# jonasrothfuss/ProMP

Measured on AMD Instinct MI355X. Metric: env-steps/sec through GAE+inner+outer update, higher is better.
Workload: dtype f32

## Files before the change

include/promp_hip.h:

```cpp
#ifndef PROMP_HIP_H
#define PROMP_HIP_H

#include <stddef.h>
#include <stdint.h>

#ifdef __cplusplus
extern "C" {
#endif

typedef struct promp_ctx promp_ctx;

typedef struct promp_dims {
    int32_t n_tasks;
    int32_t n_tasks_global;
    int32_t obs_dim;
    int32_t act_dim;
    int32_t hidden1, hidden2;
    int32_t num_inner_steps;
    int32_t max_rows;
    int32_t max_paths;
    int32_t n_hidden;
    int32_t hidden3, hidden4;
    int32_t hidden_act;
} promp_dims;
// ... 57 lines not shown
int promp_set_theta(promp_ctx* ctx, const float* theta);
int promp_get_theta(promp_ctx* ctx, float* theta);
int promp_set_step_sizes(promp_ctx* ctx, const float* step_sizes);
int promp_get_step_sizes(promp_ctx* ctx, float* step_sizes);
int promp_set_train_step_sizes(promp_ctx* ctx, int on);
int promp_get_step_size_grad(promp_ctx* ctx, float* grad);
int promp_set_step_size_adam_state(promp_ctx* ctx, const float* m, const float* v);
int promp_get_step_size_adam_state(promp_ctx* ctx, float* m, float* v);
int promp_set_learn_std(promp_ctx* ctx, int learn_std);
int promp_set_min_std(promp_ctx* ctx, float min_std);
int promp_set_schedule(promp_ctx* ctx, int stage_overlap, int fuse_min_tasks);
int promp_set_primal_cache(promp_ctx* ctx, int on);
int promp_set_reuse_adapt(promp_ctx* ctx, int on);
long long promp_adapt_passes_skipped(promp_ctx* ctx);
long long promp_constraint_hvp_cached_passes(promp_ctx* ctx);
long long promp_state_version(promp_ctx* ctx);
int promp_set_adam_state(promp_ctx* ctx, const float* m, const float* v, int64_t t);
int promp_get_adam_state(promp_ctx* ctx, float* m, float* v, int64_t* t);
int promp_switch_to_pre_update(promp_ctx* ctx);
int promp_set_task_thetas(promp_ctx* ctx, const float* theta_tasks);
int promp_get_task_thetas(promp_ctx* ctx, float* theta_tasks);

int promp_inner_adapt(promp_ctx* ctx, int step, int inner_kind);

int promp_policy_forward(promp_ctx* ctx, const float* obs, int batch, float* mean_out);

int promp_begin_rollout(promp_ctx* ctx, int step, int envs_per_task, int path_length);
int promp_begin_collection(promp_ctx* ctx, int step, int envs_per_task, int max_steps);
int promp_end_collection(promp_ctx* ctx, int step, int n_paths, const int32_t* task_path_offsets, const int32_t* path_env,
                         const int32_t* path_start, const int32_t* path_len, const float* rewards);
// ... 59 lines not shown
```

promp_amd/_lib.py:

```python
import ctypes as C
import os

import weakref

import numpy as np

_HERE = os.path.dirname(os.path.abspath(__file__))
DEFAULT_LIBRARY = os.path.join(_HERE, 'libpromp_hip.so')

BASELINE_ZERO, BASELINE_LINEAR_FEATURE, BASELINE_LINEAR_TIME = 0, 1, 2
INNER_RATIO, INNER_LOGLIK, INNER_DICE = 0, 1, 2
OUTER_CLIP, OUTER_RATIO, OUTER_KL, OUTER_LOGLIK = 0, 1, 2, 3
LOSS_RATIO, LOSS_CLIP, LOSS_LOGLIK, LOSS_KL = 0, 1, 2, 3
KERNEL_FWD_BWD, KERNEL_HVP, KERNEL_GRAM, KERNEL_FWD, KERNEL_EXCHANGE = 0, 1, 2, 3, 4


class PrompError(RuntimeError):
    pass


class Dims(C.Structure):
    _fields_ = [('n_tasks', C.c_int32), ('n_tasks_global', C.c_int32), ('obs_dim', C.c_int32), ('act_dim', C.c_int32),
                ('hidden1', C.c_int32), ('hidden2', C.c_int32), ('num_inner_steps', C.c_int32),
                ('max_rows', C.c_int32), ('max_paths', C.c_int32),
# ... 34 lines not shown
    'promp_predict_baseline': (C.c_int, [_P, C.c_int, C.c_int, _D]),
    'promp_set_advantages': (C.c_int, [_P, C.c_int, _F]),
    'promp_set_theta': (C.c_int, [_P, _F]),
    'promp_get_theta': (C.c_int, [_P, _F]),
    'promp_set_step_sizes': (C.c_int, [_P, _F]),
    'promp_get_step_sizes': (C.c_int, [_P, _F]),
    'promp_set_train_step_sizes': (C.c_int, [_P, C.c_int]),
    'promp_get_step_size_grad': (C.c_int, [_P, _F]),
    'promp_set_step_size_adam_state': (C.c_int, [_P, _F, _F]),
    'promp_get_step_size_adam_state': (C.c_int, [_P, _F, _F]),
    'promp_set_learn_std': (C.c_int, [_P, C.c_int]),
    'promp_set_primal_cache': (C.c_int, [_P, C.c_int]),
    'promp_set_reuse_adapt': (C.c_int, [_P, C.c_int]),
    'promp_adapt_passes_skipped': (C.c_longlong, [_P]),
    'promp_constraint_hvp_cached_passes': (C.c_longlong, [_P]),
    'promp_state_version': (C.c_longlong, [_P]),
    'promp_set_min_std': (C.c_int, [_P, C.c_float]),
    'promp_set_schedule': (C.c_int, [_P, C.c_int, C.c_int]),
    'promp_set_rewards_f64': (C.c_int, [_P, C.c_int, _D]),
    'promp_stage_step': (C.c_int, [_P, C.c_int, C.c_int, _I, _I, _F, _F, _F, _F, _F, C.c_int]),
    'promp_commit_step': (C.c_int, [_P, C.c_int]),
    'promp_stage_wait': (C.c_int, [_P]),
    'promp_host_alloc': (C.c_void_p, [C.c_size_t]),
    'promp_host_free': (None, [C.c_void_p]),
    'promp_constraint_hvp': (C.c_int, [_P, C.c_int, _F, C.c_int, _F]),
    'promp_cg_solve': (C.c_int, [_P, C.c_int, _F, C.c_int, C.c_float, C.c_float, C.c_int, C.c_float, _F, C.POINTER(C.c_double)]),
    'promp_set_step_selection': (C.c_int, [_P, C.c_int, C.c_int, _I]),
    'promp_step_selection': (C.c_int, [_P, C.c_int]),
    'promp_use_selection': (C.c_int, [_P, C.c_int]),
    'promp_set_adam_state': (C.c_int, [_P, _F, _F, C.c_int64]),
# ... 657 lines not shown
    def set_primal_cache(self, on=True):
        self._call('promp_set_primal_cache', -1 if on is None else int(bool(on)))

    def set_reuse_adapt(self, on=True):
        self._call('promp_set_reuse_adapt', int(bool(on)))

    def adapt_passes_skipped(self):
        return int(self.lib.cdll.promp_adapt_passes_skipped(self._h))

    def state_version(self):
        return int(self.lib.cdll.promp_state_version(self._h))

    def constraint_hvp_cached_passes(self):
        return int(self.lib.cdll.promp_constraint_hvp_cached_passes(self._h))

    def set_min_std(self, min_std):
        self._call('promp_set_min_std', float(min_std))

    def set_learn_std(self, on=True):
        self._call('promp_set_learn_std', int(bool(on)))

    def adam_step(self, lr):
        self._call('promp_adam_step', float(lr))

    def optimize(self, num_epochs, lr, clip_eps, inner_kl_coeff, inner_kind=INNER_RATIO, outer_kind=OUTER_CLIP):
        eta = _f32(inner_kl_coeff)
        assert eta.shape == (self.K,)
        lb, stats = C.c_float(0), np.empty(self.K + 2, np.float32)
        self._call('promp_optimize', int(num_epochs), float(lr), float(clip_eps), _ptr(eta, C.c_float), int(inner_kind),
                   int(outer_kind), C.byref(lb), _ptr(stats, C.c_float))
# ... 166 lines not shown
```

promp_amd/csrc/promp_hip.hip:

```cpp
#include "promp_plan.h"
#include "promp_kernels_chain.h"
#include "promp_kernels_pass.h"
#include "promp_kernels_policy.h"
#include "promp_kernels_policy_wide.h"
#include "promp_kernels_wide_bf16.h"
#include "promp_kernels_sample.h"
#include "promp_kernels_rollout.h"
#include "promp_kernels_generic.h"
#include "promp_kernels_generic_bf16.h"
#include "../../include/promp_hip.h"

#include <algorithm>
#include <cmath>
#include <cstdarg>
#include <cstdio>
#include <cstdlib>
#include <cstring>
#include <memory>
#include <string>
#include <vector>

#define PROMP_ARCH_NAME(prop) (prop).gcnArchName

namespace {
// ... 195 lines not shown
    float eta_last[PROMP_ETA_MAX] = {};
    DevBuf<double> gram_partials, red64;
    DevBuf<char> rollout_buf;
    DevBuf<float> stage_rows;
    DevBuf<double> fit_scratch;
    size_t smem_fwd = 0, smem_hvp = 0;
    PlanSwitches sw;
    PassFamily family = PassFamily::Chain;
    int wb_cls = 0;
    size_t smem_wb_fwd = 0, smem_wb_bwd = 0, smem_wb_hvp = 0;
    DevBuf<unsigned> wb_planes, wb_vplanes;
    DevBuf<unsigned> wb_planes_meta;
    DevBuf<float> cg_buf;
    DevBuf<double> cg_scal;
    struct { bool valid = false; unsigned long long theta_version = 0, data_version = 0, sizes_version = 0; const void* step = nullptr; } wbp;
    DevBuf<unsigned> vdir_absmax;
    int gramt_map_nblk = -1;
    GramtMap gramt_map;
    bool gen_bf16 = true;
    DevBuf<unsigned short> gb_wplanes, gb_vplanes;
    long long gb_plane_stride = 0;
    int gb_pf_off[GEN_MAX_LIN] = {}, gb_pb_off[GEN_MAX_LIN] = {};
    int n_lin = 0, g_maxw = 0;
    GenLin lin[GEN_MAX_LIN];
    DevBuf<float> g_act[GEN_MAX_LIN], g_ract[GEN_MAX_LIN], g_mu, g_rmu, g_dz[2], g_qz[2];
    DevBuf<unsigned long long> dbg;
    bool dbg_enabled = false;
    DevBuf<int> task_counters;
    DevBuf<int> split_events;
    ncclComm_t comm = nullptr;
// ... 228 lines not shown
    const int slices = (c->n_cus * 2 + c->d.n_tasks - 1) / c->d.n_tasks;
    PROMP_LAUNCH(k_obs_range, dim3(slices < 1 ? 1 : slices > 32 ? 32 : slices, c->d.n_tasks), 256, 16, st, r);
    HIPCHECK(hipGetLastError());
    S.obs_range_valid = true;
    c->wbp.valid = false;
    return 0;
}

static bool primal_cache_on(const promp_ctx* c) { return c->family == PassFamily::Chain && c->primal_cache != 0; }
static int ensure_primal_cache(promp_ctx* c, StepData& S) {
    if (S.hcache) return 0;
    const size_t rows = S.cap_rows ? S.cap_rows : c->d.max_rows;
    return S.hcache.alloc((rows + 16 * (size_t)c->d.n_tasks) * chain_cache_row(c->d.hidden1, c->d.hidden2));
}

static void launch_chain(promp_ctx* c, StepData& S, const PassArgs& a, const PassReq& q, int cache) {
    const int n1 = c->d.hidden1 / 16, n2 = c->d.hidden2 / 16, ks = chain_ksteps(c->d.obs_dim);
    const dim3 grid(S.n_chain_wg);
    if (q.hvp) {
#define PROMP_CHAIN_CASE(N1, N2, KS)                                                                                             \
    if (n1 == N1 && n2 == N2 && ks == KS) {                                                                                      \
        if (cache == 2) { auto k = k_chain_hvp<N1, N2, KS, CHAIN_NW_HVP, true>; PROMP_LAUNCH(k, grid, 64 * CHAIN_NW_HVP, c->smem_hvp, c->stream, a); } \
        else { auto k = k_chain_hvp<N1, N2, KS, CHAIN_NW_HVP, false>; PROMP_LAUNCH(k, grid, 64 * CHAIN_NW_HVP, c->smem_hvp, c->stream, a); }           \
    }
        PROMP_CHAIN_ALL(PROMP_CHAIN_CASE)
#undef PROMP_CHAIN_CASE
        return;
    }
#define PROMP_PASS_CASE(N1, N2)                                                                                                          \
    if (n1 == N1 && n2 == N2) {                                                                                                          \
        if (q.fwd_only) { auto k = k_pass<N1, N2, CHAIN_NW_HVP, false, false>; PROMP_LAUNCH(k, grid, 64 * CHAIN_NW_HVP, c->smem_fwd, c->stream, a); }   \
        else if (cache == 1) { auto k = k_pass<N1, N2, CHAIN_NW_HVP, true, true>; PROMP_LAUNCH(k, grid, 64 * CHAIN_NW_HVP, c->smem_fwd, c->stream, a); } \
        else { auto k = k_pass<N1, N2, CHAIN_NW_HVP, true, false>; PROMP_LAUNCH(k, grid, 64 * CHAIN_NW_HVP, c->smem_fwd, c->stream, a); }            \
    }
    PROMP_PASS_ALL(PROMP_PASS_CASE)
#undef PROMP_PASS_CASE
}

static void launch_coop_fp32(promp_ctx* c, StepData& S, const PassArgs& a, const PassReq& q) {
    const int nob = wide_nob(c->d.obs_dim);
    const size_t sm = q.hvp ? c->smem_hvp : c->smem_fwd;
#define PROMP_WIDE_CASE(HH, NOB)                                                                                                \
    if (c->d.hidden1 == HH && nob == NOB) {                                                                                      \
        if (q.hvp) { auto k = k_wide_hvp<HH, NOB>; PROMP_LAUNCH(k, dim3(S.n_work[0]), 4 * HH, sm, c->stream, a); }               \
        else if (q.fwd_only) { auto k = k_wide_fwd_bwd<HH, NOB, false>; PROMP_LAUNCH(k, dim3(S.n_work[0]), 4 * HH, sm, c->stream, a); } \
        else { auto k = k_wide_fwd_bwd<HH, NOB, true>; PROMP_LAUNCH(k, dim3(S.n_work[0]), 4 * HH, sm, c->stream, a); }            \
    }
    PROMP_WIDE_ALL(PROMP_WIDE_CASE)
#undef PROMP_WIDE_CASE
}
// ... 53 lines not shown
    a.segs = S.chain_segs; a.wg_seg_offsets = S.chain_wg_offsets;
    a.theta = q.theta; a.theta_task_stride = q.theta_stride;
    a.vdir = c->vbuf;
    a.partials = c->partials; a.partial_stride = c->partial_stride;
    a.O = c->d.obs_dim; a.A = c->d.act_dim;
    a.loss_kind = q.loss_kind; a.clip_eps = q.clip_eps; a.clip_log_std = q.clip_ls;
    a.min_log_std = c->min_log_std;
    a.kl_weight = q.klw;
    a.task_counters = c->task_counters; a.task_slot_offsets = S.chain_slot_offsets;
    a.fuse_reduce = (q.hvp && chain && c->d.n_tasks >= c->fuse_min_tasks) ? 1 : 0;
    float* scal = q.scal ? q.scal : c->scal_tmp;
    a.red_mode = q.red_mode; a.step_sizes = c->step_sizes; a.cur = q.cur; a.cur_task_stride = q.cur_stride; a.next = q.next;
    a.lam = c->lam; a.v = c->vbuf; a.scal = scal;
    a.dbg = c->dbg_enabled ? c->dbg.p : nullptr;
    a.split_events = c->split_events;
    const int id = q.hvp ? PROMP_KERNEL_HVP : q.fwd_only ? PROMP_KERNEL_FWD : PROMP_KERNEL_FWD_BWD;
    if (prof_begin(c, id, S.n_rows)) return -2;
    switch (c->family) {
    case PassFamily::Chain: launch_chain(c, S, a, q, cache); break;
    case PassFamily::CoopFp32: launch_coop_fp32(c, S, a, q); break;
    case PassFamily::CoopSplit: launch_coop_split(c, S, a, q); break;
    case PassFamily::Layered: if (launch_pass_generic(c, S, a, q.hvp, q.fwd_only)) return -2; break;
    }
    HIPCHECK(hipGetLastError());
    if (prof_end(c, id)) return -2;
    if (a.fuse_reduce) return 0;
    ReduceArgs r;
    r.partials = c->partials; r.partial_stride = c->partial_stride;
    r.task_wg_offsets = chain ? S.chain_slot_offsets : S.task_wg_offsets[0];
    r.NP = c->NP;
// ... 139 lines not shown
    ad.stats = c->stats + (size_t)c->stats_slot * (K + 2); ad.NP = NP; ad.K = K; ad.A = c->d.act_dim;
    for (int k = 0; k < PROMP_ETA_MAX; ++k) ad.eta[k] = k < K ? eta_host[k] : 0.f;
    ad.host_stats = c->publish_next ? c->stats_host.p : nullptr; ad.host_seq = c->stats_seq_host; ad.seq = c->stats_seq;
    ad.inv_tasks = 1.0f / (float)c->d.n_tasks_global;
    ad.do_update = do_adam ? 1 : 0;
    ad.n_trainable = c->learn_std ? NP : NP - c->d.act_dim;
    ad.lr_t = 0.f;
    if (do_adam) {
        c->theta_version = ++c->version_counter;
        if (ag) c->sizes_version = ++c->version_counter;
        c->ls_known = false;
        c->adam_t += 1;
        const double t = (double)c->adam_t;
        ad.lr_t = (float)((double)lr * std::sqrt(1.0 - std::pow(0.999, t)) / (1.0 - std::pow(0.9, t)));
    }
    if (ag) {
        const StepSizeArgs ss = step_size_args(c);
        if (split) PROMP_LAUNCH(k_mean_adam_ss, dim3((2 * NP + 1 + 255) / 256), 256, 0, c->stream, ad, ss);
        else PROMP_LAUNCH(k_final_adam_ss, dim3(final_blocks + 1), 256, 0, c->stream, f, ad, ss);
    } else if (split) PROMP_LAUNCH(k_mean_adam, dim3((NP + 1 + 255) / 256), 256, 0, c->stream, ad);
    else PROMP_LAUNCH(k_final_adam, dim3(final_blocks + 1), 256, 0, c->stream, f, ad);
    HIPCHECK(hipGetLastError());
    for (int k = 0; k <= K; ++k) W[k].dirty = true;
    return 0;
}
int enqueue_meta(promp_ctx* c, float clip_eps, const float* eta_host, int inner_kind, int outer_kind, bool want_grad,
                 bool do_adam, float lr, bool sizes_grad = true) {
    return enqueue_meta_on(c, full_set(c), clip_eps, eta_host, inner_kind, outer_kind, want_grad, do_adam, lr, sizes_grad);
}

// ... 197 lines not shown
        c->smem_fwd = sizeof(float) * (size_t)pass_layout(dims->hidden1 / 16, dims->hidden2 / 16, CHAIN_NW_HVP, c->NP).total;
        c->smem_hvp = sizeof(float) * (size_t)std::max(chain_layout(dims->hidden1 / 16, dims->hidden2 / 16, CHAIN_NW_HVP, true, c->NP).total,
                                                       chain_layout(dims->hidden1 / 16, dims->hidden2 / 16, CHAIN_NW_HVP, true, c->NP, true).total);
        break;
    }
    if (c->smem_hvp > 160 * 1024 || c->smem_fwd > 160 * 1024) {
        const size_t need = c->smem_hvp > c->smem_fwd ? c->smem_hvp : c->smem_fwd;
        return fail(-1, "LDS budget exceeded (%zu bytes)", need);
    }
    {
        const int lds = 160 * 1024;
#define PROMP_CHAIN_LDS(N1, N2, KS) if (allow_lds(lds, k_chain_hvp<N1, N2, KS, CHAIN_NW_HVP, false>, k_chain_hvp<N1, N2, KS, CHAIN_NW_HVP, true>)) return -2;
        PROMP_CHAIN_ALL(PROMP_CHAIN_LDS)
#undef PROMP_CHAIN_LDS
#define PROMP_PASS_LDS(N1, N2) \
    if (allow_lds(lds, k_pass<N1, N2, CHAIN_NW_HVP, true, true>, k_pass<N1, N2, CHAIN_NW_HVP, true, false>, k_pass<N1, N2, CHAIN_NW_HVP, false, false>)) return -2;
        PROMP_PASS_ALL(PROMP_PASS_LDS)
#undef PROMP_PASS_LDS
#define PROMP_WB_LDS(CLS, NKO, NXB) if (allow_lds(lds, k_wb_hvp<NKO, NXB>, k_wb_fwd_bwd<NKO, NXB, true>, k_wb_fwd_bwd<NKO, NXB, false>)) return -2;
        PROMP_WB_ALL(PROMP_WB_LDS)
#undef PROMP_WB_LDS
#define PROMP_WIDE_LDS(HH, NOB) if (allow_lds(lds, k_wide_fwd_bwd<HH, NOB, true>, k_wide_fwd_bwd<HH, NOB, false>, k_wide_hvp<HH, NOB>)) return -2;
        PROMP_WIDE_ALL(PROMP_WIDE_LDS)
#undef PROMP_WIDE_LDS
#define PROMP_GEN_LDS(NBW)                                                                                                   \
    if (allow_lds(lds, k_gen_linear<GEN_FWD, NBW>, k_gen_linear<GEN_FWD_T, NBW>, k_gen_linear<GEN_BWD, NBW>, k_gen_linear<GEN_BWD_T, NBW>, \
                  k_gen_wgrad<1, NBW>, k_gen_wgrad<2, NBW>, k_gb_linear<GEN_FWD, NBW>, k_gb_linear<GEN_FWD_T, NBW>,            \
                  k_gb_linear<GEN_BWD, NBW>, k_gb_linear<GEN_BWD_T, NBW>, k_gb_wgrad<1, NBW>, k_gb_wgrad<2, NBW>)) return -2;
        PROMP_GEN_LDS(1) PROMP_GEN_LDS(2) PROMP_GEN_LDS(3) PROMP_GEN_LDS(4)
#undef PROMP_GEN_LDS
        if (allow_lds((int)gen_loss_smem(GEN_MAX_A), k_gen_loss<true, true>, k_gen_loss<false, true>, k_gen_loss<false, false>)) return -2;
#define PROMP_GRAM_INST(NBLK) k_gram<NBLK>,
#define PROMP_FITWV_INST(DT) k_fit_wave<DT>,
        if (allow_lds(lds, PROMP_GRAM_ALL(PROMP_GRAM_INST) PROMP_FITWV_ALL(PROMP_FITWV_INST) k_fit, k_gram_wide, k_gram_tiled<GRAMT_TB, GRAMT_NWV, GRAMT_NLD>, k_fitw_panel<32>, k_fitw_panel<16>,
                      k_fitw_update<32>, k_fitw_update<16>, k_fitw_back<32>, k_fitw_back<16>, k_fit_wide<32>, k_fit_wide<16>)) return -2;
#undef PROMP_GRAM_INST
#undef PROMP_FITWV_INST
    }
    const size_t NP = c->NP, MNP = (size_t)M * NP;
    if (c->theta.alloc(NP) || c->step_sizes.alloc(NP)) return -2;
    if (c->adam_m.alloc(NP) || c->adam_v.alloc(NP)) return -2;
    if (c->theta_tasks.alloc(MNP) || c->chain.alloc((size_t)(K + 1) * MNP)) return -2;
    if (c->lam.alloc(MNP) || c->vbuf.alloc(MNP)) return -2;
    if (c->family == PassFamily::CoopSplit) {
        const size_t pw = (size_t)M * wb_planes_words(wb_nko(c->wb_cls));
        if (c->wb_planes.alloc(pw) || c->wb_vplanes.alloc(pw) || c->wb_planes_meta.alloc(pw)) return -2;
        if (c->vdir_absmax.alloc((size_t)M)) return -2;
    }
    if (c->partials.alloc((size_t)c->max_work * c->partial_stride)) return -2;
    if (c->scal_inner.alloc((size_t)K * M * 2) || c->scal_outer.alloc((size_t)M * 2)) return -2;
    if (c->scal_tmp.alloc((size_t)M * 2)) return -2;
    if (c->red.alloc(NP + K + 2) || c->grad_mean.alloc(NP)) return -2;
    if (c->stats.alloc((size_t)2 * (K + 2))) return -2;
    if (c->red64.alloc(64)) return -2;
    if (c->family == PassFamily::Layered) {
        const size_t R = (size_t)dims->max_rows;
        for (int l = 1; l < c->n_lin; ++l)
            if (c->g_act[l].alloc(R * c->lin[l].K) || c->g_ract[l].alloc(R * c->lin[l].K)) return -2;
// ... 540 lines not shown
    if (stage_overlap >= 0) {
        HIPCHECK(hipStreamSynchronize(c->side));
        c->overlap = stage_overlap != 0;
    }
    if (fuse_min_tasks >= 0) c->fuse_min_tasks = fuse_min_tasks;
    return 0;
}
int promp_set_reuse_adapt(promp_ctx* c, int on) {
    NEED_CTX(c);
    c->reuse_adapt = on != 0;
    c->adapt0.valid = false;
    return 0;
}
long long promp_adapt_passes_skipped(promp_ctx* c) { return c ? c->adapt_passes_skipped : -1; }
long long promp_constraint_hvp_cached_passes(promp_ctx* c) { return c ? c->chvp_cached_passes : -1; }
long long promp_state_version(promp_ctx* c) { return c ? (long long)c->version_counter : -1; }
int promp_set_primal_cache(promp_ctx* c, int on) {
    NEED_CTX(c);
    c->primal_cache = on < 0 ? -1 : on != 0;
    return 0;
}
int promp_set_learn_std(promp_ctx* c, int on) {
    NEED_CTX(c);
    if (on && !c->learn_std) return fail(-3, "learn_std cannot be switched back on: the log_std step sizes were zeroed (set the step sizes again)");
    c->learn_std = on != 0;
    c->sizes_version = ++c->version_counter;
    return mask_log_std_step_sizes(c);
}
static int tasks_materialize(promp_ctx* c);
int promp_set_task_thetas(promp_ctx* c, const float* t) {
// ... 506 lines not shown
    AdamArgs ad;
    ad.theta = c->theta; ad.m = c->adam_m; ad.v = c->adam_v; ad.red = c->red; ad.grad_mean = c->grad_mean;
    ad.stats = c->stats; ad.NP = c->NP; ad.K = c->d.num_inner_steps;
    for (int k = 0; k < PROMP_ETA_MAX; ++k) ad.eta[k] = k < ad.K ? c->eta_last[k] : 0.f;
    ad.host_stats = nullptr; ad.host_seq = nullptr; ad.seq = 0;
    ad.inv_tasks = 1.0f / (float)c->d.n_tasks_global;
    ad.do_update = 1;
    ad.n_trainable = c->learn_std ? c->NP : c->NP - c->d.act_dim;
    ad.A = c->d.act_dim;
    c->theta_version = ++c->version_counter;
    if (c->train_sizes) c->sizes_version = ++c->version_counter;
    c->ls_known = false;
    c->adam_t += 1;
    const double t = (double)c->adam_t;
    ad.lr_t = (float)((double)lr * std::sqrt(1.0 - std::pow(0.999, t)) / (1.0 - std::pow(0.9, t)));
    if (c->train_sizes) PROMP_LAUNCH(k_mean_adam_ss, dim3((2 * c->NP + 1 + 255) / 256), 256, 0, c->stream, ad, step_size_args(c));
    else PROMP_LAUNCH(k_mean_adam, dim3((c->NP + 1 + 255) / 256), 256, 0, c->stream, ad);
    HIPCHECK(hipGetLastError());
    return 0;
}

int promp_optimize_begin(promp_ctx* c, int num_epochs, float lr, float clip_eps, const float* eta, int inner_kind, int outer_kind) {
    if (!c || !eta) return fail(-1, "NULL argument");
    if (num_epochs < 0) return fail(-1, "num_epochs must be >= 0");
    if (c->opt_pending) return fail(-1, "promp_optimize_begin: the previous optimisation has not been collected (promp_optimize_end)");
    if (sharded_without_comm(c))
        return fail(-3, "this context holds %d of %d tasks and has no communicator: promp_optimize would apply this rank's sums as if they "
                        "were the meta-batch's.  Attach one (promp_comm_init), or run the exchange yourself: promp_meta_grad -> "
                        "promp_reduced_get -> all-reduce -> promp_reduced_set -> promp_adam_step", c->d.n_tasks, c->d.n_tasks_global);
    if (upload_eta(c, eta)) return -2;
// ... 256 lines not shown
```

promp_amd/csrc/promp_kernels_chain.h:

```cpp
#pragma once
#include "promp_device.h"
#include "promp_objective.h"
#include "promp_plan.h"

#define PROMP_PASS_TPLANE 512
#define PROMP_PASS_XPLANE 256
#define PROMP_PASS_DPLANE 160
#define PROMP_PARTIAL_EXTRA 4
#define PROMP_CH_TS 68
#define PROMP_CH_DS 20
#define PROMP_CH_ROW 68
#define PROMP_CH_BLK (4 * PROMP_CH_ROW)

#ifndef PROMP_PASS_XCD
#define PROMP_PASS_XCD 0
#endif

PROMP_CX int chain_cache_row(int H1, int H2) { return 2 * H1 + H2 + 8; }


enum { RED_STEP = 0, RED_OUTER = 1, RED_HVP = 2, RED_PLAIN = 3, RED_SCAL = 4 };

struct PassArgs {
    const float* obs;
// ... 25 lines not shown
    const float* step_sizes;
    const float* cur;
    long long cur_task_stride;
    float* next;
    float* lam;
    float* v;
    float* scal;
    float* row_tan;
    float* hcache;
    unsigned long long* dbg;
    int* split_events;
    const float* vdir_absmax;
    const unsigned* wb_theta_planes;
    const unsigned* wb_v_planes;
    long long wb_plane_stride;
};


struct ChainLds {
    int w1, w2, w3, w3b, b1, b2, b3, dist;
    int net_stride;
    int planes, plane_stride;
    int bplanes, bplane_stride;
    int flag;
    int wave0, wave_stride, tb0, tb1, db0, db1;
    int tp, tq, tah, xt, dm0, dm1;
    int vmx;
    int total;
};
#define PROMP_CH_TPL 512
// ... 1411 lines not shown
```

promp_amd/csrc/promp_kernels_pass.h:

```cpp
#pragma once
#include "promp_device.h"
#include "promp_kernels_chain.h"


struct PassLds {
    int wp, plane_stride;
    int f_w1, f_w2f, f_w2b, f_w3f, n_frag;
    int w3b, b1, b2, b3, dist, n_side;
    int wave0, wave_stride, xt, ta, tb, dm;
    int total;
};

PROMP_CX PassLds pass_layout(int NC1, int NC2, int nwaves, int NP) {
    PassLds L{};
    int o = 4;
    L.f_w1 = 0;
    L.f_w2f = L.f_w1 + NC1 * 64;
    L.f_w2b = L.f_w2f + NC2 * (NC1 / 2) * 64;
    L.f_w3f = L.f_w2b + NC1 * (NC2 / 2) * 64;
    L.n_frag = L.f_w3f + (NC2 / 2) * 64;
    L.plane_stride = 4 * L.n_frag;
    L.wp = o; o += PROMP_NT * L.plane_stride;
    L.w3b = o; o += NC2 * 128;
    L.b1 = o; o += 16 * NC1;
// ... 135 lines not shown
        const int bj = w + it * NW;
        put(x3[it], B2 + (bj < NK3 ? bj : NK3 - 1), 1.f, 1.f);
    }
#pragma unroll
    for (int it = 0; it < IT4; ++it) {
        const int bj = w + it * NW;
        put(x4[it], B3 + (bj < NK4 ? bj : NK4 - 1), aok ? 1.f : 0.f, aok ? 1.f : 0.f);
    }
#pragma unroll
    for (int it = 0; it < IS; ++it) {
        const int ej = tid + it * NT, e = ej < L.n_side ? ej : L.n_side - 1;
        sm[L.w3b + e] = y[it];
    }
}

template <int NC1, int NC2, int NW>
PROMP_DEV bool pass_reduce_to_partial(float* S, float* P, const f32x16 (&aw2)[NC1 / 2][NC2 / 2], const f32x16 (&aw1)[NC1 / 2],
                                      const f32x4 (&aw3)[NC2], const f32x4 (&gb1)[NC1], const f32x4 (&gb2)[NC2], float gs0,
                                      float gs1, float gb30, float gb31, float loss, float klsum, int O, int A, int tid, float gsc,
                                      float gsc1, int bad) {
    constexpr int H1 = 16 * NC1, H2 = 16 * NC2, NT = 64 * NW;
    tid += opaque_zero();
    const int lane = tid & 63, w = tid >> 6, i16 = lane & 15, kk = lane >> 4, j32 = lane & 31, kh = lane >> 5;
    const Mlp2Layout lay = mlp2_layout(O, H1, H2, A);
    const int SL = (lay.NP + 2 + 3) & ~3;
    if (lane == 0) ((int*)S)[w - 4] = bad;
    lds_barrier();
    {
        float* mine = S + w * SL;
#pragma unroll
// ... 400 lines not shown
        PROMP_SCHED_MFMA(1);
        PROMP_SCHED_VALU(PROMP_NT == 3 ? 6 : 7);
        PROMP_SCHED_DSWRITE(1);
    }
    sched_fence();
    PASS_STAMP(9);
#pragma unroll
    for (int tt = 0; tt < PROMP_NT; ++tt) Q.fx[tt] = fx[tt];
#pragma unroll
    for (int b = 0; b < NB1; ++b) pass_read_tr(Q.fd[b], TA, TPL, T.rd32_0 + 256 * b, T.rd32_1 + 256 * b);
    pass_load_frags<NC1>(w1f, F, PS, L.f_w1, 64);
    sched_fence();
    PASS_STAMP(10);
}

template <int NC1, int NC2, int NW, bool BWD, bool STORE>
__global__ void __launch_bounds__(64 * NW, NW / 4) k_pass(PassArgs a) {
    constexpr int H1 = 16 * NC1, H2 = 16 * NC2, NB1 = NC1 / 2, NB2 = NC2 / 2;
    constexpr int DPL = PROMP_PASS_DPLANE;
    constexpr PassLds L = pass_layout(NC1, NC2, NW, 0);
    PROMP_SMEM_DECL;
    float* sm = (float*)PROMP_SMEM_PTR;
    const int tid = threadIdx.x, lane = tid & 63, w = wave_uniform(tid >> 6);
    const int i16 = lane & 15, kk = lane >> 4;
    const int O = a.O, A = a.A;
    const Mlp2Layout lay = mlp2_layout(O, H1, H2, A);
    const float* dist = sm + L.dist;
    float* wreg = sm + L.wave0 + w * L.wave_stride;
    const PassTileAddr T = pass_tile_addr(lane);
    PassWalk W;
    W.obs = a.obs; W.act = a.act; W.adv = a.adv; W.old_mean = a.old_mean; W.old_log_std = a.old_log_std; W.hcache = a.hcache;
// ... 14 lines not shown
        W.tnrows = a.task_row_offsets[seg.task + 1] - W.trow0;
        W.invN = 1.0f / (float)W.tnrows;
        W.tend = seg.tile0 + seg.ntiles;
        const float* th = a.theta + (long long)seg.task * a.theta_task_stride;
        float xr[8];
        int t = seg.tile0 + w;
        const ChainDistRaw draw = chain_dist_load(th, nullptr, lay.ls, A, tid);
        CH_STAMP(0);
        float w1s = 1.f;
        W.xs = 1.f;
        {
            const int sx = obs_shift(a.obs_absmax, seg.task);
            W.xs = pow2f(-sx);
            w1s = pow2f(sx);
        }
        pass_stage_net<NC1, NC2, NW>(sm, th, O, A, tid, w1s, [&]() {
            pass_load_x(xr, W, t, i16, kk);
            __syncthreads();
        });
        chain_stage_dist(sm + L.dist, draw, A, a.clip_log_std, a.min_log_std, tid);
        for (int e = lane; e < PROMP_NT * DPL; e += 64) wreg[L.dm + e] = 0.f;
        __syncthreads();
        CH_STAMP(1);
        W.s0 = dist[CH_LS + W.q0]; W.s1 = dist[CH_LS + W.q1]; W.e0 = dist[CH_ES + W.q0]; W.e1 = dist[CH_ES + W.q1];
        W.sn20 = dist[CH_SN2 + W.q0]; W.sn21 = dist[CH_SN2 + W.q1]; W.rden0 = dist[CH_RDEN + W.q0]; W.rden1 = dist[CH_RDEN + W.q1];
        W.sums = 0.f;
        for (int aa = 0; aa < A; ++aa) W.sums += dist[CH_LS + aa];

        PassSums<NC1, NC2> S;
#pragma unroll
        for (int i = 0; i < NB1; ++i) {
#pragma unroll
            for (int r = 0; r < 16; ++r) S.aw1[i][r] = 0.f;
#pragma unroll
// ... 142 lines not shown
```

promp_amd/csrc/promp_kernels_policy.h:

```cpp
#pragma once
#include "promp_device.h"
#include "promp_kernels_chain.h"
#include "promp_kernels_pass.h"
#include "promp_kernels_step_sizes.h"

struct ReduceArgs {
    const float* partials;
    int partial_stride;
    const int* task_wg_offsets;
    int NP;
    const float* step_sizes;
    int mode;
    const float* cur;
    long long cur_task_stride;
    float* next;
    float* lam;
    float* v;
    float* scal;
    float* next2;
    float* scal2;
};

template <bool KEEP_G>
PROMP_DEV void reduce_task_body(const ReduceArgs& a, float* ginner) {
// ... 101 lines not shown
    float* theta;
    float* m;
    float* v;
    const float* red;
    float* grad_mean;
    float* stats;
    float eta[PROMP_ETA_MAX];
    int NP, K, A;
    float inv_tasks;
    float lr_t;
    int do_update;
    int n_trainable;
    float* host_stats;
    unsigned* host_seq;
    unsigned seq;
};
PROMP_DEV void publish_stats(const AdamArgs& a) {
    if (a.host_stats == nullptr) return;
    for (int i = 0; i < 2 * (a.K + 2); ++i) a.host_stats[i] = a.stats[i];
    {
        float lo = a.theta[a.NP - a.A];
        for (int i = 1; i < a.A; ++i) lo = fminf(lo, a.theta[a.NP - a.A + i]);
        a.host_stats[2 * (a.K + 2)] = lo;
    }
    release_store_system(a.host_seq, a.seq);
}

template <bool SS>
PROMP_DEV void mean_adam_body(const AdamArgs& a, const StepSizeArgs& ss) {
    const int j = blockIdx.x * 256 + threadIdx.x;
    if (j < a.NP) {
        const float g = a.red[j] * a.inv_tasks;
        a.grad_mean[j] = g;
        if (a.do_update && j < a.n_trainable) {
            const float m = 0.9f * a.m[j] + 0.1f * g;
            const float v = 0.999f * a.v[j] + 0.001f * g * g;
            a.m[j] = m;
            a.v[j] = v;
            a.theta[j] -= a.lr_t * m / (sqrtf(v) + 1e-8f);
        }
    } else if (j == a.NP) {
        float pen = 0.f;
        for (int k = 0; k < a.K; ++k) {
            const float ikl = a.red[a.NP + 1 + k] * a.inv_tasks;
            a.stats[1 + k] = ikl;
            pen += a.eta[k] * ikl;
        }
        a.stats[0] = a.red[a.NP] * a.inv_tasks + pen / (float)a.K;
        a.stats[1 + a.K] = a.red[a.NP + 1 + a.K] * a.inv_tasks;
        publish_stats(a);
    } else if (SS && j <= 2 * a.NP) {
        const int ja = j - a.NP - 1;
        step_size_adam(ss.alpha, ss.alpha_m, ss.alpha_v, ss.alpha_grad_mean, ja, a.red[a.NP + a.K + 2 + ja] * a.inv_tasks,
                       a.do_update && ja < a.n_trainable, ja < a.n_trainable, a.lr_t);
    }
// ... 4 lines not shown
__global__ void __launch_bounds__(256) k_sum_ranks(const float* gathered, float* out, int n, int nranks) {
    const int j = blockIdx.x * 256 + threadIdx.x;
    if (j >= n) return;
    float s = gathered[j];
    for (int r = 1; r < nranks; ++r) s += gathered[(long long)r * n + j];
    out[j] = s;
}

template <bool SS>
PROMP_DEV void final_adam_body(const FinalArgs& a, const AdamArgs& ad, const StepSizeArgs& ss, float (*part)[64], float* sums) {
    const int c = threadIdx.x & 63, q = threadIdx.x >> 6;
    const bool stats_block = blockIdx.x == gridDim.x - 1;
    const int j = stats_block ? a.NP + c : blockIdx.x * 64 + c;
    const int jend = a.NP + a.K + 2 + (SS && !stats_block ? a.NP : 0);
    float s = 0.f;
    if (j < a.NP) {
        if (a.want_grad) s = final_quarter_sum(a.lam, a.NP, a.n_tasks, j, q);
    } else if (j == a.NP) {
        for (int i = q; i < a.n_tasks; i += 4) s += a.scal_outer[i * 2 + 0];
    } else if (j <= a.NP + a.K) {
        const int k = j - a.NP - 1;
        for (int i = q; i < a.n_tasks; i += 4) s += a.scal_inner[((long long)k * a.n_tasks + i) * 2 + 1];
    } else if (j == a.NP + a.K + 1) {
        for (int i = q; i < a.n_tasks; i += 4) s += a.scal_outer[i * 2 + 1];
    } else if (SS && j < jend) {
        s = final_quarter_sum(ss.galpha, a.NP, a.n_tasks, j - (a.NP + a.K + 2), q);
    }
    part[q][c] = s;
    __syncthreads();
    if (q == 0 && j < jend) {
        const float t = (part[0][c] + part[1][c]) + (part[2][c] + part[3][c]);
        if (!stats_block) a.red[j] = t;
        sums[c] = t;
        if (!stats_block && j < a.NP) {
            const float g = t * ad.inv_tasks;
            ad.grad_mean[j] = g;
            if (ad.do_update && j < ad.n_trainable) {
                const float m = 0.9f * ad.m[j] + 0.1f * g;
                const float v = 0.999f * ad.v[j] + 0.001f * g * g;
                ad.m[j] = m;
                ad.v[j] = v;
                ad.theta[j] -= ad.lr_t * m / (sqrtf(v) + 1e-8f);
            }
        } else if (SS && !stats_block && j >= a.NP + a.K + 2) {
            const int ja = j - (a.NP + a.K + 2);
            step_size_adam(ss.alpha, ss.alpha_m, ss.alpha_v, ss.alpha_grad_mean, ja, t * ad.inv_tasks,
                           ad.do_update && ja < ad.n_trainable, ja < ad.n_trainable, ad.lr_t);
        }
    }
    if (!stats_block) return;
    __syncthreads();
    if (threadIdx.x == 0) {
        float pen = 0.f;
        for (int k = 0; k < a.K; ++k) {
            const float ikl = sums[1 + k] * ad.inv_tasks;
            ad.stats[1 + k] = ikl;
            pen += ad.eta[k] * ikl;
        }
// ... 145 lines not shown
```

promp_amd/csrc/promp_plan.h:

```cpp
#pragma once
#include "../../include/promp_hip.h"

#include <algorithm>
#include <cmath>
#include <cstdarg>
#include <cstdio>
#include <cstdlib>
#include <cstring>
#include <string>
#include <vector>

#ifdef __HIPCC__
#define PROMP_PLAN_HD __host__ __device__ inline
#else
#define PROMP_PLAN_HD inline
#endif

inline int plan_fail(std::string* why, int code, const char* fmt, ...) {
    char buf[1024];
    va_list ap;
    va_start(ap, fmt);
    vsnprintf(buf, sizeof buf, fmt, ap);
    va_end(ap);
    if (why) *why = buf;
    return code;
}

struct PlanSwitches {
    bool fit_one_launch = false;
    bool gram_untiled = false;
    bool gramt_single = false;
    bool wide_fp32 = false;
    bool gen_fp32 = false;
    int max_cus = 0;
};
inline PlanSwitches plan_switches_from_env() {
    auto is1 = [](const char* name) { const char* e = getenv(name); return e && e[0] == '1'; };
    PlanSwitches sw;
    sw.fit_one_launch = is1("PROMP_FIT_ONE_LAUNCH");
    sw.gram_untiled = is1("PROMP_GRAM_UNTILED");
    sw.gramt_single = is1("PROMP_GRAMT_SINGLE");
    sw.gen_fp32 = is1("PROMP_GEN_FP32");
    { const char* e = getenv("PROMP_WIDE_FP32"); sw.wide_fp32 = e && atoi(e) != 0; }
    { const char* e = getenv("PROMP_MAX_CUS"); sw.max_cus = e ? atoi(e) : 0; }
    return sw;
}

#define GEN_MAX_LIN 5
#define GEN_MAX_N 256
#define GEN_MAX_A 64
#define PROMP_ETA_MAX 8
#define PROMP_LINFEAT_MAX_O 480

constexpr int CHAIN_NW_HVP = 4;
inline int chain_ksteps(int obs_dim) { return obs_dim <= 8 ? 2 : obs_dim <= 20 ? 5 : 8; }
inline int wide_nob(int obs_dim) { return obs_dim <= 32 ? 2 : obs_dim <= 64 ? 4 : 8; }
inline int wb_nko(int cls) { return cls == 1 ? 4 : cls == 2 ? 7 : 8; }

struct HiddenList {
// ... 416 lines not shown
```

Before: 293.7 million.

## Prebuild split-precision parameter plane image in Adam update for chain passes

```diff
diff --git a/include/promp_hip.h b/include/promp_hip.h
--- a/include/promp_hip.h
+++ b/include/promp_hip.h
@@ -95,6 +95,7 @@
 int promp_set_reuse_adapt(promp_ctx* ctx, int on);
 long long promp_adapt_passes_skipped(promp_ctx* ctx);
 long long promp_constraint_hvp_cached_passes(promp_ctx* ctx);
+long long promp_param_plane_passes(promp_ctx* ctx);
 long long promp_state_version(promp_ctx* ctx);
 int promp_set_adam_state(promp_ctx* ctx, const float* m, const float* v, int64_t t);
 int promp_get_adam_state(promp_ctx* ctx, float* m, float* v, int64_t* t);
diff --git a/promp_amd/_lib.py b/promp_amd/_lib.py
--- a/promp_amd/_lib.py
+++ b/promp_amd/_lib.py
@@ -72,6 +72,7 @@
     'promp_set_reuse_adapt': (C.c_int, [_P, C.c_int]),
     'promp_adapt_passes_skipped': (C.c_longlong, [_P]),
     'promp_constraint_hvp_cached_passes': (C.c_longlong, [_P]),
+    'promp_param_plane_passes': (C.c_longlong, [_P]),
     'promp_state_version': (C.c_longlong, [_P]),
     'promp_set_min_std': (C.c_int, [_P, C.c_float]),
     'promp_set_schedule': (C.c_int, [_P, C.c_int, C.c_int]),
@@ -759,6 +760,9 @@
     def constraint_hvp_cached_passes(self):
         return int(self.lib.cdll.promp_constraint_hvp_cached_passes(self._h))
 
+    def param_plane_passes(self):
+        return int(self.lib.cdll.promp_param_plane_passes(self._h))
+
     def set_min_std(self, min_std):
         self._call('promp_set_min_std', float(min_std))
 
diff --git a/promp_amd/csrc/promp_hip.hip b/promp_amd/csrc/promp_hip.hip
--- a/promp_amd/csrc/promp_hip.hip
+++ b/promp_amd/csrc/promp_hip.hip
@@ -233,6 +233,10 @@
     DevBuf<float> cg_buf;
     DevBuf<double> cg_scal;
     struct { bool valid = false; unsigned long long theta_version = 0, data_version = 0, sizes_version = 0; const void* step = nullptr; } wbp;
+    int pp_words = 0;
+    DevBuf<unsigned> pp_meta;
+    struct { bool valid = false; unsigned long long theta_version = 0; } pp_meta_rec;
+    long long pp_passes = 0;
     DevBuf<unsigned> vdir_absmax;
     int gramt_map_nblk = -1;
     GramtMap gramt_map;
@@ -491,6 +495,17 @@
     return S.hcache.alloc((rows + 16 * (size_t)c->d.n_tasks) * chain_cache_row(c->d.hidden1, c->d.hidden2));
 }
 
+static PlaneImage plane_image(const promp_ctx* c, unsigned* img) {
+    PlaneImage I;
+    I.img = img; I.O = c->d.obs_dim; I.NC1 = c->d.hidden1 / 16; I.NC2 = c->d.hidden2 / 16; I.A = c->d.act_dim;
+    return I;
+}
+static PlaneImage plane_image_meta(promp_ctx* c) {
+    if (!c->pp_words || (c->pp_meta_rec.valid && c->pp_meta_rec.theta_version == c->theta_version)) return plane_image(c, nullptr);
+    c->pp_meta_rec.valid = true; c->pp_meta_rec.theta_version = c->theta_version;
+    return plane_image(c, c->pp_meta.p);
+}
+
 static void launch_chain(promp_ctx* c, StepData& S, const PassArgs& a, const PassReq& q, int cache) {
     const int n1 = c->d.hidden1 / 16, n2 = c->d.hidden2 / 16, ks = chain_ksteps(c->d.obs_dim);
     const dim3 grid(S.n_chain_wg);
@@ -504,13 +519,16 @@
 #undef PROMP_CHAIN_CASE
         return;
     }
-#define PROMP_PASS_CASE(N1, N2)                                                                                                          \
-    if (n1 == N1 && n2 == N2) {                                                                                                          \
-        if (q.fwd_only) { auto k = k_pass<N1, N2, CHAIN_NW_HVP, false, false>; PROMP_LAUNCH(k, grid, 64 * CHAIN_NW_HVP, c->smem_fwd, c->stream, a); }   \
-        else if (cache == 1) { auto k = k_pass<N1, N2, CHAIN_NW_HVP, true, true>; PROMP_LAUNCH(k, grid, 64 * CHAIN_NW_HVP, c->smem_fwd, c->stream, a); } \
-        else { auto k = k_pass<N1, N2, CHAIN_NW_HVP, true, false>; PROMP_LAUNCH(k, grid, 64 * CHAIN_NW_HVP, c->smem_fwd, c->stream, a); }            \
-    }
-    PROMP_PASS_ALL(PROMP_PASS_CASE)
+#define PROMP_PASS_CASE(N1, N2, IMG)                                                                                                     \
+    if (n1 == N1 && n2 == N2 && img == IMG) {                                                                                            \
+        if (q.fwd_only) { auto k = k_pass<N1, N2, CHAIN_NW_HVP, false, false, IMG>; PROMP_LAUNCH(k, grid, 64 * CHAIN_NW_HVP, c->smem_fwd, c->stream, a); }   \
+        else if (cache == 1) { auto k = k_pass<N1, N2, CHAIN_NW_HVP, true, true, IMG>; PROMP_LAUNCH(k, grid, 64 * CHAIN_NW_HVP, c->smem_fwd, c->stream, a); } \
+        else { auto k = k_pass<N1, N2, CHAIN_NW_HVP, true, false, IMG>; PROMP_LAUNCH(k, grid, 64 * CHAIN_NW_HVP, c->smem_fwd, c->stream, a); }            \
+    }
+#define PROMP_PASS_CASE2(N1, N2) PROMP_PASS_CASE(N1, N2, false) PROMP_PASS_CASE(N1, N2, true)
+    const bool img = a.pimg != nullptr;
+    PROMP_PASS_ALL(PROMP_PASS_CASE2)
+#undef PROMP_PASS_CASE2
 #undef PROMP_PASS_CASE
 }
 
@@ -594,6 +612,11 @@
     a.lam = c->lam; a.v = c->vbuf; a.scal = scal;
     a.dbg = c->dbg_enabled ? c->dbg.p : nullptr;
     a.split_events = c->split_events;
+    if (chain && c->pp_words && !q.hvp && q.theta == c->theta.p && q.theta_stride == 0 && c->pp_meta_rec.valid &&
+        c->pp_meta_rec.theta_version == c->theta_version) {
+        a.pimg = c->pp_meta.p;
+        c->pp_passes += 1;
+    }
     const int id = q.hvp ? PROMP_KERNEL_HVP : q.fwd_only ? PROMP_KERNEL_FWD : PROMP_KERNEL_FWD_BWD;
     if (prof_begin(c, id, S.n_rows)) return -2;
     switch (c->family) {
@@ -763,6 +786,7 @@
         const double t = (double)c->adam_t;
         ad.lr_t = (float)((double)lr * std::sqrt(1.0 - std::pow(0.999, t)) / (1.0 - std::pow(0.9, t)));
     }
+    ad.img = plane_image_meta(c);
     if (ag) {
         const StepSizeArgs ss = step_size_args(c);
         if (split) PROMP_LAUNCH(k_mean_adam_ss, dim3((2 * NP + 1 + 255) / 256), 256, 0, c->stream, ad, ss);
@@ -990,7 +1014,8 @@
         PROMP_CHAIN_ALL(PROMP_CHAIN_LDS)
 #undef PROMP_CHAIN_LDS
 #define PROMP_PASS_LDS(N1, N2) \
-    if (allow_lds(lds, k_pass<N1, N2, CHAIN_NW_HVP, true, true>, k_pass<N1, N2, CHAIN_NW_HVP, true, false>, k_pass<N1, N2, CHAIN_NW_HVP, false, false>)) return -2;
+    if (allow_lds(lds, k_pass<N1, N2, CHAIN_NW_HVP, true, true, false>, k_pass<N1, N2, CHAIN_NW_HVP, true, false, false>, k_pass<N1, N2, CHAIN_NW_HVP, false, false, false>, \
+                  k_pass<N1, N2, CHAIN_NW_HVP, true, true, true>, k_pass<N1, N2, CHAIN_NW_HVP, true, false, true>, k_pass<N1, N2, CHAIN_NW_HVP, false, false, true>)) return -2;
         PROMP_PASS_ALL(PROMP_PASS_LDS)
 #undef PROMP_PASS_LDS
 #define PROMP_WB_LDS(CLS, NKO, NXB) if (allow_lds(lds, k_wb_hvp<NKO, NXB>, k_wb_fwd_bwd<NKO, NXB, true>, k_wb_fwd_bwd<NKO, NXB, false>)) return -2;
@@ -1018,6 +1043,10 @@
     if (c->adam_m.alloc(NP) || c->adam_v.alloc(NP)) return -2;
     if (c->theta_tasks.alloc(MNP) || c->chain.alloc((size_t)(K + 1) * MNP)) return -2;
     if (c->lam.alloc(MNP) || c->vbuf.alloc(MNP)) return -2;
+    if (c->family == PassFamily::Chain && c->sw.param_planes) {
+        c->pp_words = pass_image_words(c->d.hidden1 / 16, c->d.hidden2 / 16);
+        if (c->pp_meta.alloc((size_t)c->pp_words)) return -2;
+    }
     if (c->family == PassFamily::CoopSplit) {
         const size_t pw = (size_t)M * wb_planes_words(wb_nko(c->wb_cls));
         if (c->wb_planes.alloc(pw) || c->wb_vplanes.alloc(pw) || c->wb_planes_meta.alloc(pw)) return -2;
@@ -1588,6 +1617,7 @@
 }
 long long promp_adapt_passes_skipped(promp_ctx* c) { return c ? c->adapt_passes_skipped : -1; }
 long long promp_constraint_hvp_cached_passes(promp_ctx* c) { return c ? c->chvp_cached_passes : -1; }
+long long promp_param_plane_passes(promp_ctx* c) { return c ? c->pp_passes : -1; }
 long long promp_state_version(promp_ctx* c) { return c ? (long long)c->version_counter : -1; }
 int promp_set_primal_cache(promp_ctx* c, int on) {
     NEED_CTX(c);
@@ -2124,6 +2154,7 @@
     c->adam_t += 1;
     const double t = (double)c->adam_t;
     ad.lr_t = (float)((double)lr * std::sqrt(1.0 - std::pow(0.999, t)) / (1.0 - std::pow(0.9, t)));
+    ad.img = plane_image_meta(c);
     if (c->train_sizes) PROMP_LAUNCH(k_mean_adam_ss, dim3((2 * c->NP + 1 + 255) / 256), 256, 0, c->stream, ad, step_size_args(c));
     else PROMP_LAUNCH(k_mean_adam, dim3((c->NP + 1 + 255) / 256), 256, 0, c->stream, ad);
     HIPCHECK(hipGetLastError());
diff --git a/promp_amd/csrc/promp_kernels_chain.h b/promp_amd/csrc/promp_kernels_chain.h
--- a/promp_amd/csrc/promp_kernels_chain.h
+++ b/promp_amd/csrc/promp_kernels_chain.h
@@ -63,6 +63,7 @@
     const unsigned* wb_theta_planes;
     const unsigned* wb_v_planes;
     long long wb_plane_stride;
+    const unsigned* pimg;
 };
 
 
diff --git a/promp_amd/csrc/promp_kernels_pass.h b/promp_amd/csrc/promp_kernels_pass.h
--- a/promp_amd/csrc/promp_kernels_pass.h
+++ b/promp_amd/csrc/promp_kernels_pass.h
@@ -173,6 +173,111 @@
     }
 }
 
+PROMP_CX int pass_image_words(int NC1, int NC2) {
+    const PassLds L = pass_layout(NC1, NC2, 1, 0);
+    return L.dist - L.wp;
+}
+struct PlaneImage {
+    unsigned* img;
+    int O, NC1, NC2, A;
+};
+PROMP_DEV void pass_image_put(unsigned* img, const PassLds& L, int frag, int e, float x) {
+    unsigned w[PROMP_NT];
+    split_pair<PROMP_NT>(x, x, w);
+    unsigned short* h = (unsigned short*)img;
+#pragma unroll
+    for (int t = 0; t < PROMP_NT; ++t) h[2 * (t * L.plane_stride + 4 * frag + (e >> 1)) + (e & 1)] = (unsigned short)(w[t] & 0xffffu);
+}
+PROMP_DEV void pass_image_file(const PlaneImage& I, int j, float x) {
+    const int NC1 = I.NC1, NC2 = I.NC2, A = I.A, H2 = 16 * NC2, NP1 = NC1 / 2, NP2 = NC2 / 2;
+    const PassLds L = pass_layout(NC1, NC2, 1, 0);
+    const Mlp2Layout lay = mlp2_layout(I.O, 16 * NC1, H2, A);
+    if (j < lay.b1 || j >= lay.ls) return;
+    unsigned* img = I.img;
+    float* side = (float*)img + (L.w3b - L.wp);
+    int P, kk, e;
+    auto slot = [&](int u) { P = u >> 5; kk = (u >> 2) & 3; e = 4 * ((u >> 4) & 1) + (u & 3); };
+    if (j < lay.W2) {
+        side[L.b1 - L.w3b + (j - lay.b1)] = x * PROMP_TANH_PRESCALE;
+    } else if (j < lay.b2) {
+        const int u1 = (j - lay.W2) >> (NC2 == 4 ? 6 : 5), u2 = (j - lay.W2) - u1 * H2;
+        slot(u1);
+        pass_image_put(img, L, L.f_w2f + 64 * ((u2 >> 4) * NP1 + P) + 16 * kk + (u2 & 15), e, x * PROMP_TANH_PRESCALE);
+        slot(u2);
+        pass_image_put(img, L, L.f_w2b + 64 * ((u1 >> 4) * NP2 + P) + 16 * kk + (u1 & 15), e, x * 1.f);
+    } else if (j < lay.W3) {
+        side[L.b2 - L.w3b + (j - lay.b2)] = x * PROMP_TANH_PRESCALE;
+    } else if (j < lay.b3) {
+        const int u = (j - lay.W3) / A, aa = (j - lay.W3) - u * A;
+        slot(u);
+        const int fr = L.f_w3f + 64 * P + 16 * kk;
+        pass_image_put(img, L, fr + 4 * (aa >> 1) + (aa & 1), e, x * 1.f);
+        const int sb = (u >> 4) * 128 + 2 * (u & 15);
+        side[sb + 32 * (aa >> 1) + (aa & 1)] = x * 1.f;
+        if (aa == 0) {
+            const float z = x * 0.f;
+            for (int i16 = 0; i16 < 16; ++i16) {
+                const int ro = i16 & 3;
+                if (!(ro < 2 && 2 * (i16 >> 2) + ro < A)) pass_image_put(img, L, fr + i16, e, z);
+            }
+            for (int p = A; p < 8; ++p) side[sb + 32 * (p >> 1) + (p & 1)] = z;
+        }
+    } else {
+        const int aa = j - lay.b3;
+        side[L.b3 - L.w3b + aa] = x * 1.f;
+        if (aa == 0)
+            for (int p = A; p < 8; ++p) side[L.b3 - L.w3b + p] = x * 0.f;
+    }
+}
+
+template <int NC1, int NC2, int NW, typename Mid>
+PROMP_DEV void pass_stage_image(float* sm, const float* th, const unsigned* img, int O, int tid, float w1s, Mid&& mid) {
+    constexpr int H1 = 16 * NC1, NT = 64 * NW;
+    constexpr PassLds L = pass_layout(NC1, NC2, 1, 0);
+    constexpr int NK1 = L.f_w2f / 64, IT1 = (NK1 + NW - 1) / NW;
+    constexpr int NF = L.n_frag - L.f_w2f;
+    static_assert(L.n_side % 4 == 0 && L.wp % 4 == 0, "the image is copied in 16-byte units");
+    constexpr int NU = PROMP_NT * NF + L.n_side / 4, IU = (NU + NT - 1) / NT;
+    const int lane = tid & 63, i16 = lane & 15, kk = lane >> 4, w = wave_uniform(tid >> 6);
+    auto word = [&](int it) {
+        const int uj = tid + it * NT, u = uj < NU ? uj : NU - 1, t = u / NF;
+        return u < PROMP_NT * NF ? t * L.plane_stride + 4 * (L.f_w2f + (u - t * NF)) : PROMP_NT * L.plane_stride + 4 * (u - PROMP_NT * NF);
+    };
+    float x1[IT1][8];
+    u32x4 q[IU];
+#pragma unroll
+    for (int it = 0; it < IT1; ++it) {
+        const int bj = w + it * NW, b = bj < NK1 ? bj : NK1 - 1;
+#pragma unroll
+        for (int e = 0; e < 8; ++e) {
+            const int o = 8 * kk + e;
+            x1[it][e] = th[(o < O ? o : 0) * H1 + 16 * b + i16];
+        }
+    }
+#pragma unroll
+    for (int it = 0; it < IU; ++it) q[it] = *(const u32x4*)(img + word(it));
+    sched_fence();
+    mid();
+    sched_fence();
+    const float w1p = PROMP_TANH_PRESCALE * w1s;
+#pragma unroll
+    for (int it = 0; it < IT1; ++it) {
+        const int bj = w + it * NW, b = bj < NK1 ? bj : NK1 - 1;
+        f32x4 lo, hi;
+#pragma unroll
+        for (int e = 0; e < 4; ++e) {
+            lo[e] = x1[it][e] * (8 * kk + e < O ? w1p : 0.f);
+            hi[e] = x1[it][4 + e] * (8 * kk + 4 + e < O ? w1p : 0.f);
+        }
+        u32x4 pl[PROMP_NT];
+        pass_split8(lo, hi, pl);
+#pragma unroll
+        for (int t = 0; t < PROMP_NT; ++t) sts_w4(sm + L.wp + t * L.plane_stride + 4 * (64 * b + lane), pl[t]);
+    }
+#pragma unroll
+    for (int it = 0; it < IU; ++it) sts_w4(sm + L.wp + word(it), q[it]);
+}
+
 template <int NC1, int NC2, int NW>
 PROMP_DEV bool pass_reduce_to_partial(float* S, float* P, const f32x16 (&aw2)[NC1 / 2][NC2 / 2], const f32x16 (&aw1)[NC1 / 2],
                                       const f32x4 (&aw3)[NC2], const f32x4 (&gb1)[NC1], const f32x4 (&gb2)[NC2], float gs0,
@@ -603,7 +708,7 @@
     PASS_STAMP(10);
 }
 
-template <int NC1, int NC2, int NW, bool BWD, bool STORE>
+template <int NC1, int NC2, int NW, bool BWD, bool STORE, bool IMG>
 __global__ void __launch_bounds__(64 * NW, NW / 4) k_pass(PassArgs a) {
     constexpr int H1 = 16 * NC1, H2 = 16 * NC2, NB1 = NC1 / 2, NB2 = NC2 / 2;
     constexpr int DPL = PROMP_PASS_DPLANE;
@@ -648,10 +753,12 @@
             W.xs = pow2f(-sx);
             w1s = pow2f(sx);
         }
-        pass_stage_net<NC1, NC2, NW>(sm, th, O, A, tid, w1s, [&]() {
+        auto mid = [&]() {
             pass_load_x(xr, W, t, i16, kk);
             __syncthreads();
-        });
+        };
+        if constexpr (IMG) pass_stage_image<NC1, NC2, NW>(sm, th, a.pimg, O, tid, w1s, mid);
+        else pass_stage_net<NC1, NC2, NW>(sm, th, O, A, tid, w1s, mid);
         chain_stage_dist(sm + L.dist, draw, A, a.clip_log_std, a.min_log_std, tid);
         for (int e = lane; e < PROMP_NT * DPL; e += 64) wreg[L.dm + e] = 0.f;
         __syncthreads();
diff --git a/promp_amd/csrc/promp_kernels_policy.h b/promp_amd/csrc/promp_kernels_policy.h
--- a/promp_amd/csrc/promp_kernels_policy.h
+++ b/promp_amd/csrc/promp_kernels_policy.h
@@ -139,6 +139,7 @@
     float* host_stats;
     unsigned* host_seq;
     unsigned seq;
+    PlaneImage img;
 };
 PROMP_DEV void publish_stats(const AdamArgs& a) {
     if (a.host_stats == nullptr) return;
@@ -155,6 +156,7 @@
 PROMP_DEV void mean_adam_body(const AdamArgs& a, const StepSizeArgs& ss) {
     const int j = blockIdx.x * 256 + threadIdx.x;
     if (j < a.NP) {
+        float th = a.theta[j];
         const float g = a.red[j] * a.inv_tasks;
         a.grad_mean[j] = g;
         if (a.do_update && j < a.n_trainable) {
@@ -162,8 +164,10 @@
             const float v = 0.999f * a.v[j] + 0.001f * g * g;
             a.m[j] = m;
             a.v[j] = v;
-            a.theta[j] -= a.lr_t * m / (sqrtf(v) + 1e-8f);
-        }
+            th -= a.lr_t * m / (sqrtf(v) + 1e-8f);
+            a.theta[j] = th;
+        }
+        if (a.img.img != nullptr) pass_image_file(a.img, j, th);
     } else if (j == a.NP) {
         float pen = 0.f;
         for (int k = 0; k < a.K; ++k) {
@@ -198,6 +202,8 @@
     const int j = stats_block ? a.NP + c : blockIdx.x * 64 + c;
     const int jend = a.NP + a.K + 2 + (SS && !stats_block ? a.NP : 0);
     float s = 0.f;
+    float th = 0.f;
+    if (q == 0 && !stats_block && j < a.NP) th = ad.theta[j];
     if (j < a.NP) {
         if (a.want_grad) s = final_quarter_sum(a.lam, a.NP, a.n_tasks, j, q);
     } else if (j == a.NP) {
@@ -224,8 +230,10 @@
                 const float v = 0.999f * ad.v[j] + 0.001f * g * g;
                 ad.m[j] = m;
                 ad.v[j] = v;
-                ad.theta[j] -= ad.lr_t * m / (sqrtf(v) + 1e-8f);
+                th -= ad.lr_t * m / (sqrtf(v) + 1e-8f);
+                ad.theta[j] = th;
             }
+            if (ad.img.img != nullptr) pass_image_file(ad.img, j, th);
         } else if (SS && !stats_block && j >= a.NP + a.K + 2) {
             const int ja = j - (a.NP + a.K + 2);
             step_size_adam(ss.alpha, ss.alpha_m, ss.alpha_v, ss.alpha_grad_mean, ja, t * ad.inv_tasks,
diff --git a/promp_amd/csrc/promp_plan.h b/promp_amd/csrc/promp_plan.h
--- a/promp_amd/csrc/promp_plan.h
+++ b/promp_amd/csrc/promp_plan.h
@@ -33,6 +33,7 @@
     bool wide_fp32 = false;
     bool gen_fp32 = false;
     int max_cus = 0;
+    bool param_planes = true;
 };
 inline PlanSwitches plan_switches_from_env() {
     auto is1 = [](const char* name) { const char* e = getenv(name); return e && e[0] == '1'; };
@@ -43,6 +44,7 @@
     sw.gen_fp32 = is1("PROMP_GEN_FP32");
     { const char* e = getenv("PROMP_WIDE_FP32"); sw.wide_fp32 = e && atoi(e) != 0; }
     { const char* e = getenv("PROMP_MAX_CUS"); sw.max_cus = e ? atoi(e) : 0; }
+    { const char* e = getenv("PROMP_PARAM_PLANES"); sw.param_planes = !(e && e[0] == '0'); }
     return sw;
 }
 
```

After: 296.5 million, median of 6. No clear change (+1.0%).
